# mmheyer/a3-reliable-transport

Hardware: AMD Instinct MI355X
Metric: GiB/s CRC-32 over device-resident 1456-B payloads; % of HBM read roofline (higher is better)
Workload: dtype u8

## Files before the change

a3-reliable-transport_amd/csrc/crc32_kernels.hip:

```cpp
#include <hip/hip_runtime.h>

#include <algorithm>
#include <atomic>
#include <cstdarg>
#include <cstdint>
#include <cstdio>
#include <cstdlib>
#include <cstring>
#include <mutex>
#include <type_traits>
#include <unordered_map>
#include <string>
#include <vector>

#include "crc32_math.hpp"
#include "wtp_crc32.h"

namespace wtp {

constexpr int kG = 16;
constexpr int kBraids = 4 * kG;
constexpr uint32_t kBraidBlock = 4 * kBraids;
#ifndef WTP_PC_S
#define WTP_PC_S 64
// ... 131 lines not shown
            for (int k = 0; k < PER; ++k)
                v[k] = sets[(k * THREADS) >> 11].g[stag_fill_word((uint32_t(k * THREADS) + threadIdx.x) & 2047u)];
        }
    }
    __device__ __forceinline__ void store(char *lds, const StagSet (&sets)[NS]) const {
        if constexpr (kX4) {
#pragma unroll
            for (int k = 0; k < PER; ++k) {
                const uint32_t sidx = (uint32_t(k * THREADS) + threadIdx.x) & 511u;
                uint32_t soff;
                if constexpr (THREADS <= 512) {
                    soff = sets[(k * THREADS) >> 9].off;
                } else {
                    const uint32_t si = (uint32_t(k * THREADS) + threadIdx.x) >> 9;
                    soff = sets[0].off;
#pragma unroll
                    for (int i = 1; i < NS; ++i) soff = si == uint32_t(i) ? sets[i].off : soff;
                }
                const uint32_t base = soff + (sidx >> 3) * 1024u + ((sidx >> 1) & 3u) * 32u + (sidx & 1u) * 16u;
#pragma unroll
                for (uint32_t i = 0; i < 4; ++i)
                    *reinterpret_cast<u32x4 *>(lds + base + i * 256u) = u32x4{v[k][i], v[k][i], v[k][i], v[k][i]};
            }
        } else {
#pragma unroll
            for (int k = 0; k < PER; ++k) {
                const uint32_t j = (uint32_t(k * THREADS) + threadIdx.x) & 2047u;
                *reinterpret_cast<u32x4 *>(lds + sets[(k * THREADS) >> 11].off + stag_fill_off(j)) =
                    u32x4{v[k], v[k], v[k], v[k]};
            }
        }
    }
};
template <int NS, int THREADS>
__device__ __forceinline__ void fill_stag_batch(char *lds, const StagSet (&sets)[NS]) {
    StagFill<NS, THREADS> f;
    f.load(sets);
    f.store(lds, sets);
}

__device__ __forceinline__ uint32_t braid_lead(uintptr_t st, uint32_t len, uint32_t frame) {
    const uint32_t l128 = uint32_t(st & 127u), l64 = uint32_t(st & 63u);
    return l128 + len <= frame ? l128 : (l64 + len <= frame ? l64 : frame - len);
}

__device__ __forceinline__ uint32_t xor3(uint32_t a, uint32_t b, uint32_t c) {
    return __builtin_amdgcn_bitop3_b32(a, b, c, 0x96);
}

template <uint32_t OFF>
__device__ __forceinline__ uint32_t stag_apply3x(const char *lds, const uint32_t (&key)[4], const uint32_t (&sel)[4],
                                                 uint32_t x, uint32_t w) {
    const uint32_t a0 = __builtin_amdgcn_perm(x, key[0], sel[0]);
    const uint32_t a1 = __builtin_amdgcn_perm(x, key[1], sel[1]);
    const uint32_t a2 = __builtin_amdgcn_perm(x, key[2], sel[2]);
    const uint32_t a3 = __builtin_amdgcn_perm(x, key[3], sel[3]);
    return xor3(xor3(lds_rd(lds, a0 + OFF), lds_rd(lds, a1 + OFF), lds_rd(lds, a2 + OFF)), lds_rd(lds, a3 + OFF), w);
}

template <uint32_t OFF>
__device__ __forceinline__ uint32_t stag_apply3(const char *lds, const uint32_t (&key)[4], const uint32_t (&sel)[4],
                                                uint32_t x) {
    const uint32_t a0 = __builtin_amdgcn_perm(x, key[0], sel[0]);
    const uint32_t a1 = __builtin_amdgcn_perm(x, key[1], sel[1]);
    const uint32_t a2 = __builtin_amdgcn_perm(x, key[2], sel[2]);
    const uint32_t a3 = __builtin_amdgcn_perm(x, key[3], sel[3]);
    return xor3(lds_rd(lds, a0 + OFF), lds_rd(lds, a1 + OFF), lds_rd(lds, a2 + OFF)) ^ lds_rd(lds, a3 + OFF);
}

__device__ __forceinline__ uint32_t nib_apply(const char *lds, uint32_t base, uint32_t v) {
    uint32_t l[8];
#pragma unroll
    for (uint32_t i = 0; i < 8; ++i) l[i] = lds_rd(lds, base + 64u * i + 4u * __builtin_amdgcn_ubfe(v, 4 * i, 4));
    return xor3(xor3(l[0], l[1], l[2]), xor3(l[3], l[4], l[5]), l[6] ^ l[7]);
}

__device__ __forceinline__ void rotate_prio(uint32_t x) {
    switch (x & 3u) {
    case 0: __builtin_amdgcn_s_setprio(0); break;
    case 1: __builtin_amdgcn_s_setprio(1); break;
    case 2: __builtin_amdgcn_s_setprio(2); break;
    default: __builtin_amdgcn_s_setprio(3); break;
    }
}

struct CrcBEpi {
    static constexpr bool kCopy = false;
    static constexpr bool kFixup = false;
    static constexpr int kThreads = 512;
    static constexpr int kDepth = 2;
    static constexpr int kDiag = 0;
    static constexpr int kBound = 1024;
    static constexpr int kLoadAux = 2;
    static constexpr bool kHold = false;
    static constexpr const char *kName = "CrcBEpi";
    __device__ __forceinline__ uint32_t lead(uint64_t, uint32_t st, uint32_t len, uint32_t frame) const {
        return braid_lead(st, len, frame);
    }
    uint32_t *out;
    uint32_t cinit;
    struct Pre {};
    __device__ __forceinline__ void pre(uint64_t, Pre &) const {}
    __device__ __forceinline__ bool listed(bool, const Pre &) const { return false; }
    __device__ __forceinline__ void put(uint64_t p, uint32_t v, bool on, const Pre &) const {
        if (on) out[p] = v ^ cinit;
    }
};
struct CrcHoldBEpi : CrcBEpi {
    static constexpr bool kHold = true;
    static constexpr const char *kName = "CrcHoldBEpi";
};
struct VerifyBEpi {
    static constexpr bool kHold = false;
    static constexpr const char *kName = "VerifyBEpi";
    static constexpr bool kCopy = false;
    static constexpr bool kFixup = true;
    static constexpr int kThreads = 512;
    static constexpr int kDepth = 2;
    static constexpr int kDiag = 0;
    static constexpr int kBound = 1024;
    static constexpr int kLoadAux = 2;
    __device__ __forceinline__ uint32_t lead(uint64_t, uint32_t st, uint32_t len, uint32_t frame) const {
        return braid_lead(st, len, frame);
    }
    const uint32_t *rl;
    const uint8_t *ring;
    uint64_t stride;
    uint8_t *ok;
    uint32_t *crc;
    uint32_t *status;
    uint32_t cinit;
    uint64_t n;
    uint32_t full;
    struct Pre {
        uint32_t r, h;
    };
    __device__ __forceinline__ void pre(uint64_t p, Pre &q) const {
        typedef const __attribute__((address_space(1))) uint32_t gu32;
        const uint64_t pc = p < n ? p : n - 1;
        q.r = ((gu32 *)rl)[pc];
        q.h = *(gu32 *)((gu8 *)ring + pc * stride + 12);
    }
    __device__ __forceinline__ bool listed(bool on, const Pre &q) const { return on && q.r != full; }
    __device__ __forceinline__ void put(uint64_t p, uint32_t v, bool on, const Pre &q) const {
        if (!on) return;
        const uint32_t c = v ^ cinit;
        const bool mine = q.r == full;
        ok[p] = mine && bswap32(q.h) == c ? 1 : 0;
        if (crc) crc[p] = mine ? c : 0u;
    }
};

__device__ __forceinline__ __amdgpu_buffer_rsrc_t make_rsrc(const void *base, uint32_t nbytes);
#ifndef WTP_BUILD_THREADS
#define WTP_BUILD_THREADS 128
#endif
#ifndef WTP_BUILD_DIAG
#define WTP_BUILD_DIAG 0
#endif
#ifndef WTP_BUILD_DEPTH
#define WTP_BUILD_DEPTH 2
#endif
#ifndef WTP_BUILD_SAUX
#define WTP_BUILD_SAUX 2
#endif
#ifndef WTP_BUILD_WLEAD
#define WTP_BUILD_WLEAD 1
#endif
#ifndef WTP_BUILD_LAUX
#define WTP_BUILD_LAUX 2
#endif
#ifndef WTP_BUILD_SAUX0
#define WTP_BUILD_SAUX0 0
#endif
struct BuildBEpi {
    static constexpr bool kHold = false;
    static constexpr const char *kName = "BuildBEpi";
    static constexpr bool kCopy = true;
    static constexpr bool kFixup = false;
    static constexpr int kThreads = WTP_BUILD_THREADS;
    static constexpr int kDepth = WTP_BUILD_DEPTH;
    static constexpr int kDiag = WTP_BUILD_DIAG;
    static constexpr int kBound = WTP_BUILD_THREADS;
    static constexpr int kLoadAux = WTP_BUILD_LAUX;
    uint8_t *wire;
    uint64_t wstride;
    uint32_t seq0, len;
    uint32_t *wire_len;
    uint32_t cinit;
    struct Pre {};
    __device__ __forceinline__ void pre(uint64_t, Pre &) const {}
    __device__ __forceinline__ uint32_t lead(uint64_t p, uint32_t st, uint32_t l, uint32_t frame) const {
        if (WTP_BUILD_WLEAD) {
            const uint32_t w = (uint32_t(reinterpret_cast<uintptr_t>(wire)) + uint32_t(p) * uint32_t(wstride) + 16u) & 63u;
            if (w + l <= frame) return w;
        }
        return braid_lead(st, l, frame);
    }
    __device__ __forceinline__ __amdgpu_buffer_rsrc_t round_rsrc(uint64_t p0) const {
        return make_rsrc(wire + p0 * wstride, uint32_t(4 * wstride));
    }
    __device__ __forceinline__ void copy(__amdgpu_buffer_rsrc_t rs, uint32_t q, int32_t rel, bool valid, u32x4 w,
                                         bool row0) const {
        const uint32_t o = valid ? q * uint32_t(wstride) + 16u + uint32_t(rel) : 0x80000000u;
        if (row0)
            __builtin_amdgcn_raw_buffer_store_b128(w, rs, int(o), 0, WTP_BUILD_SAUX0);
        else
            __builtin_amdgcn_raw_buffer_store_b128(w, rs, int(o), 0, WTP_BUILD_SAUX);
    }
    __device__ __forceinline__ bool listed(bool, const Pre &) const { return false; }
    __device__ __forceinline__ void put(uint64_t p, uint32_t v, bool on, const Pre &) const {
        if (!on) return;
        const u32x4 h = {bswap32(WTP_TYPE_DATA), bswap32(seq0 + uint32_t(p)), bswap32(len), bswap32(v ^ cinit)};
        *reinterpret_cast<u32x4 *>(wire + p * wstride) = h;
        if (wire_len) wire_len[p] = 16u + len;
    }
};

__device__ __forceinline__ void verify_fixup(char *lds, const VerifyBEpi &epi, const uint32_t *gtab, uint32_t nfix,
                                             uint64_t rstep, uint32_t wave, uint32_t lane);

template <int ROWS, int DIAG = 0, class BEpi = CrcBEpi>
__global__ __launch_bounds__(BEpi::kBound) void k_fixed_braid(const uint8_t *__restrict__ base, uint32_t stride,
                                                      uint32_t len, uint64_t n, BEpi epi,
                                                      const uint32_t *__restrict__ gtab) {
    __shared__ __attribute__((aligned(16))) uint32_t lds_w[kBraidLdsWords];
    char *lds = reinterpret_cast<char *>(lds_w);
    constexpr uint32_t kGroup = 8;

    const uint32_t lane = threadIdx.x & 63u;
    const uint32_t wave = __builtin_amdgcn_readfirstlane(threadIdx.x >> 6);
    PC_PROBE(0, __builtin_amdgcn_s_memrealtime());
    const uint32_t nwave = blockDim.x >> 6;
    const uint32_t j = lane & (kG - 1);
    const uint32_t q = lane >> 4;
    const StagKeys K(lane);

    constexpr uint32_t kFrame = 256u * ROWS;
    const uint64_t rounds = (n + 3) >> 2;
    const uint64_t rstep = uint64_t(gridDim.x) * nwave;
    const uint32_t qoff = q * stride;
    gu8 *const gbase = (gu8 *)base;

    struct Round {
        u32x4 w[ROWS];
        uint32_t lead;
    };
    auto load_round = [&](uint64_t rr, Round &R) {
        const bool live = rr < rounds;
        const uint64_t p0 = rr * 4;
        gu8 *sb = gbase + (live ? p0 * stride : 0);
        const uint64_t last = live ? n - 1 - p0 : 0;
        const uint32_t nrec = !live ? 0u : (last >= 3 ? 3u * stride + len : uint32_t(last) * stride + len);
        const __amdgpu_buffer_rsrc_t rs = make_rsrc((const void *)sb, nrec);
        const uint32_t lead = (DIAG & 64) ? kFrame - len
                                          : epi.lead(p0 + q, uint32_t(reinterpret_cast<uintptr_t>((const void *)sb)) + qoff, len, kFrame);
        R.lead = lead;
        const uint32_t fo = qoff - lead + j * 16u;
#pragma unroll
        for (int i = 0; i < ROWS; ++i) {
            uint32_t o = fo + uint32_t(i) * 256u;
            if (i == 0 || i == ROWS - 1) {
                const int32_t rel = int32_t(uint32_t(i) * 256u + j * 16u) - int32_t(lead);
                o = (rel >= 0 && rel < int32_t(len)) ? o : 0x80000000u;
            }
            if (i == 0)
                R.w[i] = __builtin_bit_cast(u32x4, __builtin_amdgcn_raw_buffer_load_b128(rs, int(o), 0, (DIAG & 32) ? BEpi::kLoadAux : 0));
            else
                R.w[i] = __builtin_bit_cast(u32x4, __builtin_amdgcn_raw_buffer_load_b128(rs, int(o), 0, BEpi::kLoadAux));
        }
    };

    lchar *const xs = (lchar *)(lds + kBraidXpose + wave * 2048u);
    uint32_t k = 0;
    uint64_t rfirst = 0;
    typename BEpi::Pre pre{};
    uint32_t nfix = 0;
    constexpr bool kDump = ((BEpi::kHold && !(DIAG & 2048)) || (DIAG & 1024)) && !BEpi::kCopy && !BEpi::kFixup;
    const bool hold = kDump && nwave <= 8;
#ifndef WTP_BR_HOLD
#define WTP_BR_HOLD 16
#endif
    constexpr uint32_t kHoldG = WTP_BR_HOLD;
    static_assert(kHoldG == 4 || kHoldG == 8 || kHoldG == 16, "hold capacity");
    lchar *const rbuf = (lchar *)(lds + kBraidXpose + (8u + wave) * 2048u);
    uint32_t dgroups = 0;
    uint64_t dfirst = 0;
    auto dump = [&]() {
        if constexpr (kDump) {
            __builtin_amdgcn_wave_barrier();
            const uint64_t pb0 = 4 * dfirst, left = n > pb0 ? n - pb0 : 0;
            const __amdgpu_buffer_rsrc_t ors =
                make_rsrc(epi.out + pb0, left >= (1ull << 29) ? 0x80000000u : uint32_t(4 * left));
#pragma unroll
            for (uint32_t t = 0; t < (kHoldG * 8 + 63) / 64; ++t) {
                const uint32_t si = lane + 64u * t;
                const u32x4 v = *(const lu32x4 *)(rbuf + si * 16u);
                const uint64_t rr = dfirst + (8u * uint64_t(si >> 3) + (si & 7u)) * rstep;
                const uint64_t pb = 4 * rr;
                const uint32_t o = uint32_t(4 * (pb - pb0));
                const bool live = (si >> 3) < dgroups && rr < rounds;
                if (__builtin_amdgcn_ballot_w64(live && pb + 4 > n) == 0) {
                    __builtin_amdgcn_raw_buffer_store_b128(v, ors, live ? int(o) : int(0x80000000u), 0, 0);
                } else {
                    __builtin_amdgcn_raw_buffer_store_b32(v.x, ors, live && pb + 0 < n ? int(o) : int(0x80000000u), 0, 0);
                    __builtin_amdgcn_raw_buffer_store_b32(v.y, ors, live && pb + 1 < n ? int(o + 4) : int(0x80000000u), 0, 0);
                    __builtin_amdgcn_raw_buffer_store_b32(v.z, ors, live && pb + 2 < n ? int(o + 8) : int(0x80000000u), 0, 0);
                    __builtin_amdgcn_raw_buffer_store_b32(v.w, ors, live && pb + 3 < n ? int(o + 12) : int(0x80000000u), 0, 0);
                }
            }
            __builtin_amdgcn_wave_barrier();
            dgroups = 0;
        }
    };
    auto group_packet = [&](uint64_t g0) { return (g0 + uint64_t(lane >> 3) * rstep) * 4 + ((lane >> 1) & 3u); };

    auto flush = [&](uint64_t next_g0, bool more) {
        __builtin_amdgcn_wave_barrier();
        const u32x4 lo = *(const lu32x4 *)(xs + lane * 32u), hi = *(const lu32x4 *)(xs + lane * 32u + 16u);
        uint32_t acc = hi.w;
        acc = stag_apply3x<0>(lds, K.kB, K.sel, acc, hi.z);
        acc = stag_apply3x<0>(lds, K.kB, K.sel, acc, hi.y);
        acc = stag_apply3x<0>(lds, K.kB, K.sel, acc, hi.x);
        acc = stag_apply3x<0>(lds, K.kB, K.sel, acc, lo.w);
        acc = stag_apply3x<0>(lds, K.kB, K.sel, acc, lo.z);
        acc = stag_apply3x<0>(lds, K.kB, K.sel, acc, lo.y);
        acc = stag_apply3x<0>(lds, K.kB, K.sel, acc, lo.x);
        const uint32_t h = lane & 1u;
        {
            const uint32_t y = stag_apply3<128>(lds, K.kB, K.sel, acc);
            acc = h ? y : acc;
        }
        const uint64_t rr = rfirst + uint64_t(lane >> 3) * rstep;
        const uint64_t p = rr * 4 + ((lane >> 1) & 3u);
        const uint32_t st = uint32_t(reinterpret_cast<uintptr_t>(base)) + uint32_t(p) * stride;
        const uint32_t t = (kFrame - len - ((DIAG & 64) ? kFrame - len : epi.lead(p, st, len, kFrame))) >> 4;
        const uint32_t tmax = (kFrame - len) >> 4;
        for (uint32_t s2 = 0; s2 < tmax; ++s2) {
            const uint32_t y = stag_apply3<0>(lds, K.kB, K.sel, acc);
            acc = s2 < t ? y : acc;
        }
        acc ^= uint32_t(__builtin_amdgcn_update_dpp(0, int(acc), 0xB1, 0xF, 0xF, false));
        if (!(DIAG & 1)) acc = stag_apply3<0>(lds, K.kA, K.sel, acc);
        const bool on = h == 0 && (lane >> 3) < k && rr < rounds && p < n;
        if constexpr (kDump) {
            if (hold) {
                if (dgroups == 0) dfirst = rfirst;
                if (h == 0)
                    *(__attribute__((address_space(3))) uint32_t *)(rbuf + (dgroups * 8u + (lane >> 3)) * 16u +
                                                                     ((lane >> 1) & 3u) * 4u) = acc ^ epi.cinit;
                if (++dgroups == kHoldG) dump();
            } else if (!(DIAG & 16)) {
                epi.put(p, acc, on, pre);
            }
        } else if (!(DIAG & 16)) {
            epi.put(p, acc, on, pre);
        }
        if constexpr (BEpi::kFixup) nfix += uint32_t(__popcll(__ballot(epi.listed(on, pre))));
        if (more) epi.pre(group_packet(next_g0), pre);
        k = 0;
    };

    auto crc_round = [&](uint64_t rr, const Round &R) {
        if constexpr (BEpi::kCopy) {
            const auto crs = epi.round_rsrc(rr * 4);
            const bool qlive = rr * 4 + q < n;
#pragma unroll
            for (int i = 0; i < ROWS; ++i) {
                const int32_t rel = int32_t(uint32_t(i) * 256u + j * 16u) - int32_t(R.lead);
                const bool in = (i == 0 || i == ROWS - 1) ? (rel >= 0 && rel < int32_t(len)) : true;
                epi.copy(crs, q, rel, in && qlive, R.w[i], i == 0);
            }
        }
        uint32_t b0 = R.w[0].x, b1 = R.w[0].y, b2 = R.w[0].z, b3 = R.w[0].w;
#pragma unroll
        for (int i = 1; i < ROWS; ++i) {
            const u32x4 w = R.w[i];
            if (DIAG & 1) {
                b0 = (b0 ^ w.x) + (b0 >> 3);
                b1 = (b1 ^ w.y) + (b1 >> 3);
                b2 = (b2 ^ w.z) + (b2 >> 3);
                b3 = (b3 ^ w.w) + (b3 >> 3);
                continue;
            }
            b0 = stag_apply3x<0>(lds, K.kA, K.sel, b0, w.x);
            b1 = stag_apply3x<0>(lds, K.kA, K.sel, b1, w.y);
            b2 = stag_apply3x<0>(lds, K.kA, K.sel, b2, w.z);
            b3 = stag_apply3x<0>(lds, K.kA, K.sel, b3, w.w);
        }
        uint32_t v;
        if (DIAG & 2) {
            v = xor3(b0, b1, b2) ^ b3;
        } else {
            v = stag_apply3x<128>(lds, K.kA, K.sel, b3, b2);
            v = stag_apply3x<128>(lds, K.kA, K.sel, v, b1);
            v = stag_apply3x<128>(lds, K.kA, K.sel, v, b0);
        }
        if (k == 0) rfirst = rr;
        *(__attribute__((address_space(3))) uint32_t *)(xs + k * 256u + lane * 4u) = v;
        if (++k == kGroup) flush(rr + rstep, true);
    };

    uint64_t r = uint64_t(blockIdx.x) * nwave + wave;
    Round A, B;
    const StagSet sets[4] = {{gtab + OFF_BRAID, 0u},
                             {gtab + OFF_INV + 0 * 1024, 128u},
                             {gtab + OFF_INV + 2 * 1024, 65536u},
                             {gtab + OFF_INV + 5 * 1024, 65536u + 128u}};
    constexpr int kT = BEpi::kThreads;
    StagFill<4, kT> fill;
    const bool batched = blockDim.x == kT;
#ifndef WTP_BR_PROLOGUE_DIAG
#define WTP_BR_PROLOGUE_DIAG 0
#endif
    if (batched && WTP_BR_PROLOGUE_DIAG == 0) fill.load(sets);
    if constexpr (WTP_BR_PROLOGUE_DIAG == 1)
        for (int kk = 0; kk < fill.PER; ++kk) fill.v[kk] = threadIdx.x + kk;
    epi.pre(group_packet(r), pre);
    load_round(r, A);
    PC_PROBE(1, __builtin_amdgcn_s_memrealtime());
    if (WTP_BR_PROLOGUE_DIAG == 2) {
    } else if (batched) {
        fill.store(lds, sets);
    } else {
        for (int q2 = 0; q2 < 4; ++q2) fill_stag(lds, sets[q2].off >> 16, (sets[q2].off >> 7) & 1u, sets[q2].g);
    }
    PC_PROBE(2, __builtin_amdgcn_s_memrealtime());
    __syncthreads();
    PC_PROBE(3, __builtin_amdgcn_s_memrealtime());

    uint32_t prio_round = wave >> 2;
    if constexpr (BEpi::kDepth == 3) {
        Round C;
        load_round(r + rstep, B);
        while (r < rounds) {
            if (!(DIAG & 4)) rotate_prio(++prio_round);
            load_round(r + 2 * rstep, C);
            crc_round(r, A);
            r += rstep;
            if (r >= rounds) break;
            load_round(r + 2 * rstep, A);
            crc_round(r, B);
            r += rstep;
            if (r >= rounds) break;
            load_round(r + 2 * rstep, B);
            crc_round(r, C);
            r += rstep;
        }
    } else {
        while (r < rounds) {
            if (!(DIAG & 4)) rotate_prio(++prio_round);
            load_round(r + rstep, B);
            crc_round(r, A);
            if (WTP_PROBE && prio_round == (wave >> 2) + 1) PC_PROBE(4, __builtin_amdgcn_s_memrealtime());
            r += rstep;
            if (r >= rounds) break;
            load_round(r + rstep, A);
            crc_round(r, B);
            r += rstep;
        }
    }
    if (k) flush(0, false);
    if constexpr (kDump) {
        if (dgroups) dump();
    }
    PC_PROBE(5, __builtin_amdgcn_s_memrealtime());
    if constexpr (BEpi::kFixup) verify_fixup(lds, epi, gtab, nfix, rstep, wave, lane);
}

__device__ __forceinline__ __amdgpu_buffer_rsrc_t make_rsrc(const void *base, uint32_t nbytes);
struct MetaRaw {
    uint64_t a;
    uint32_t b, c, d;
};
constexpr uint32_t kRunBad = 1u, kCutBad = 2u;
struct RangeDesc {
    uint64_t begin, end, rebase;
    uint32_t nbytes, bad;
};
static_assert(sizeof(RangeDesc) == 32, "RangeDesc");
template <class P>
constexpr bool kDevRange = requires { requires P::kDevRange; };
struct CrcEpi {
    static constexpr const char *kName = "CrcEpi";
    uint32_t *out;
    uint32_t n;
    __device__ __forceinline__ void rebase(uint64_t first, uint32_t cnt) {
        out += first;
        n = cnt;
    }
    __device__ __forceinline__ void put(uint64_t p, uint32_t crc, bool, uint32_t, bool on) const {
        __builtin_amdgcn_raw_buffer_store_b32(crc, make_rsrc(out, 4 * n), on ? int(4 * p) : int(0x80000000u), 0, 0);
    }
};
struct VerifyEpi {
    static constexpr const char *kName = "VerifyEpi";
    uint8_t *ok;
    uint32_t *crc;
    uint32_t n;
    __device__ __forceinline__ void put(uint64_t p, uint32_t c, bool valid, uint32_t want, bool on) const {
        const bool good = valid && want == c;
        __builtin_amdgcn_raw_buffer_store_b8(uint8_t(good ? 1 : 0), make_rsrc(ok, n), on ? int(p) : int(0x80000000u),
                                             0, 0);
        __builtin_amdgcn_raw_buffer_store_b32(valid ? c : 0u, make_rsrc(crc, crc ? 4 * n : 0u),
                                              on ? int(4 * p) : int(0x80000000u), 0, 0);
    }
};

__device__ __forceinline__ __amdgpu_buffer_rsrc_t make_rsrc(const void *base, uint32_t nbytes) {
    return __builtin_amdgcn_make_buffer_rsrc(const_cast<void *>(base), (short)0, (int)nbytes, 0x00020000);
}
__device__ __forceinline__ u32x4 buf_ld16(__amdgpu_buffer_rsrc_t r, uint32_t off) {
    return __builtin_bit_cast(u32x4, __builtin_amdgcn_raw_buffer_load_b128(r, (int)off, 0, 0));
}

#ifndef WTP_PC_THREADS
#define WTP_PC_THREADS 1024
#endif
constexpr uint32_t kPcThreads = WTP_PC_THREADS, kPcLogT = __builtin_ctz(kPcThreads), kPcWaves = kPcThreads / 64;
constexpr uint32_t kPcWords = uint32_t(kPieceS) / 4;
constexpr uint32_t kPcNOps = kPieceS == 64 ? 5 : 6;
constexpr uint32_t kPcOps = 65536;
constexpr uint32_t kPcHinit = kPcOps + kPcNOps * kOpBytes;
#ifndef WTP_PC_SPLIT
// ... 394 lines not shown
                const uint64_t k64 = uint64_t(0xFFFFFFFFu) << (uint32_t(t) & 63u);
                const uint32_t keep = (i & 1) ? uint32_t(k64 >> 32) : uint32_t(k64);
                if ((i & 1) == 0)
                    ca = stag_apply3<0>(lds, K.kA, K.sel, __builtin_amdgcn_bitop3_b32(ca, wd, keep, 0x78));
                else if (i < 15)
                    cb = stag_apply3<0>(lds, K.kA, K.sel, __builtin_amdgcn_bitop3_b32(cb, wd, keep, 0x78));
                else
                    cb = nib_apply(lds, kPcNib4, __builtin_amdgcn_bitop3_b32(cb, wd, keep, 0x78));
            }
            c = ca ^ cb;
        }
        const uint32_t hw = lds_rd(lds, kPcHinit + 4u * uint32_t(kPieceS - (vf < 0 ? 0 : vf)));
        c ^= gp == 0u ? hw : 0u;

        uint32_t W = c;
        {
            const uint32_t u = __shfl_up(W, 1);
            if constexpr (kPieceS == 64) {
                if (lp >= 1u && lane >= 1u) W = stag_apply3x<128>(lds, K.kA, K.sel, u, W);
            } else {
                if (lp >= 1u && lane >= 1u) W = op_apply_fold(lds, kPcOps, u, W);
            }
        }
#pragma unroll
        for (uint32_t dd = 2, o = 0; dd < 64; dd <<= 1, ++o) {
            const bool need = lp >= dd && lane >= dd;
            if (__builtin_amdgcn_ballot_w64(need) == 0) break;
            const uint32_t u = __shfl_up(W, dd);
            if (need) W = op_apply_fold(lds, kPcOps + (o + kPcNOps - 5) * kOpBytes, u, W);
        }
        epi.put(pout, W ^ 0xFFFFFFFFu, pvalid, paux, active && gp == pkk - 1);
        carry = partial ? __builtin_amdgcn_readlane(W, tl) : 0u;
        skip = partial ? last_gp + 1 : 0u;
        p0 = uniform64(p0n);
        if (WTP_PROBE && nrounds == 0) PC_PROBE(4, __builtin_amdgcn_s_memrealtime());
        ++nrounds;
        if constexpr (Prov::kVarLen && WTP_PC_LAG) {
            done += total;
            const uint32_t left = wpieces > done ? wpieces - done : 0u;
            const uint32_t simd = wave & 3u;
            typedef __attribute__((address_space(3))) uint32_t lu32w;
            if (lane == 0) *(lu32w *)((lchar *)lds + kPcRem + 4u * (4u * simd + (wave >> 2))) = left;
            const uint32_t other = *(const lu32w *)((lchar *)lds + kPcRem + 16u * simd + 4u * (lane & 3u));
            rotate_prio(uint32_t(__popcll(__builtin_amdgcn_ballot_w64(lane < kPcWaves / 4u && other < left))));
        } else {
            rotate_prio(nrounds + (wave >> 2));
        }
    }
    PC_PROBE(5, __builtin_amdgcn_s_memrealtime());
    PC_PROBE(6, nrounds);
    PC_PROBE(7, hi - lo);
}

template <int THREADS>
struct PcTables {
    static constexpr uint32_t kOpQ = kPcNOps * 256, kOpPer = (kOpQ + THREADS - 1) / THREADS;
    StagFill<2, THREADS> fill;
    u32x4 q[kOpPer];
    uint32_t hv;
    u32x4 n4;
    __device__ __forceinline__ static void sets(const uint32_t *gtab, StagSet (&s)[2]) {
        s[0] = {gtab + (WTP_PC_SPLIT ? OFF_S8 : OFF_S4), 0u};
        s[1] = {gtab + (kPieceS == 64 ? OFF_FWD : OFF_X64), 128u};
    }
    __device__ __forceinline__ void load(const uint32_t *gtab) {
        StagSet ss[2];
        sets(gtab, ss);
        fill.load(ss);
        const u32x4 *src = reinterpret_cast<const u32x4 *>(gtab + OFF_FWD + 1024 * (6 - kPcNOps));
#pragma unroll
        for (uint32_t k = 0; k < kOpPer; ++k) {
            const uint32_t i = threadIdx.x + k * THREADS;
            q[k] = src[i < kOpQ ? i : 0];
        }
        hv = gtab[OFF_HINIT + (threadIdx.x <= kPieceS ? threadIdx.x : 0)];
        if constexpr (WTP_PC_SPLIT)
            n4 = reinterpret_cast<const u32x4 *>(gtab + OFF_NIB + 128 * 10)[threadIdx.x & 31u];
    }
    __device__ __forceinline__ void store(char *lds, const uint32_t *gtab) const {
        StagSet ss[2];
        sets(gtab, ss);
        fill.store(lds, ss);
        u32x4 *dst = reinterpret_cast<u32x4 *>(lds + kPcOps);
#pragma unroll
        for (uint32_t k = 0; k < kOpPer; ++k) {
            const uint32_t i = threadIdx.x + k * THREADS;
            if (i < kOpQ) dst[i] = q[k];
        }
        if (threadIdx.x <= kPieceS) reinterpret_cast<uint32_t *>(lds + kPcHinit)[threadIdx.x] = hv;
        if constexpr (WTP_PC_SPLIT)
            if (threadIdx.x < 32u) reinterpret_cast<u32x4 *>(lds + kPcNib4)[threadIdx.x] = n4;
    }
};

template <class Prov, class Epi>
__global__ __launch_bounds__(kPcThreads) void k_pieces(const uint8_t *__restrict__ base_in, uint32_t nbytes_in,
                                                 Prov prov_in, uint64_t n_in, Epi epi_in,
                                                 const uint32_t *__restrict__ gtab, uint32_t *__restrict__ status) {
    __shared__ __attribute__((aligned(16))) uint32_t lds_w[kPcLdsWords];
    char *lds = reinterpret_cast<char *>(lds_w);
    Prov prov = prov_in;
    Epi epi = epi_in;
    const uint8_t *base = base_in;
    uint32_t nbytes = nbytes_in;
    uint64_t n = n_in;
    if constexpr (kDevRange<Prov>) {
        if (!prov.bind(base, nbytes, n, epi)) return;
    }
    const uint32_t nw = blockDim.x >> 6;
    const uint64_t tw = uint64_t(gridDim.x) * nw, w0 = uint64_t(blockIdx.x) * nw;
    const uint64_t g0 = n * w0 / tw, g1 = n * (w0 + nw) / tw;
    if (g0 == g1) return;
    const uint32_t lane = threadIdx.x & 63u;
    const uint32_t wave = __builtin_amdgcn_readfirstlane(threadIdx.x >> 6);
    const __amdgpu_buffer_rsrc_t rs = make_rsrc(base, nbytes);
    PC_PROBE(0, __builtin_amdgcn_s_memrealtime());
    WaveSplit split;
    PcTables<kPcThreads> tb;
    tb.load(gtab);
    if constexpr (Prov::kVarLen) split.load(prov, g0, g1);
    PC_PROBE(1, __builtin_amdgcn_s_memrealtime());
    tb.store(lds, gtab);
    uint64_t lo, hi;
    uint32_t wpieces = 0;
    if constexpr (Prov::kVarLen) {
        split.finish(prov, g0, g1, lds, wave, lane, lo, hi, wpieces);
    } else {
        lo = n * (w0 + wave) / tw;
        hi = n * (w0 + wave + 1) / tw;
    }
    MetaRaw raw{};
    if (lo < hi) pieces_meta(prov, lo, hi, lane, raw, rs);
    __syncthreads();
    PC_PROBE(2, __builtin_amdgcn_s_memrealtime());

    pieces_loop(lds, rs, prov, epi, lo, hi, wpieces, status, wave, lane, raw);
}

constexpr uint32_t kVfWaves = 8;
constexpr uint32_t kVfList = kPcStage + kVfWaves * kPcSlot;
constexpr uint32_t kVfCap = (kPcFlags - kVfList) / 4;
constexpr uint32_t kVfCtl = (kPcLdsWords * 4 + 15) & ~15u;
constexpr uint32_t kVfPer = 8;
constexpr uint32_t kVfPass = kVfWaves * 64 * kVfPer;
static_assert(kVfPass <= kVfCap && kVfCtl + 64 <= kBraidLdsWords * 4, "verify fix-up LDS");

#ifndef WTP_AB_BUILD
static_assert(WTP_PC_S == 64 && WTP_PC_THREADS == 1024 && WTP_PC_LEN128 == 1 && WTP_PC_LAG == 1 && WTP_PC_DMA == 1 &&
                  WTP_PC_TAILCLAMP == 0 && WTP_PC_SPLIT == 0,
              "product build: piece-kernel knobs must keep their shipped values");
static_assert(WTP_BR_PROLOGUE_DIAG == 0 && WTP_PROBE == 0, "product build: no probe / prologue ablation");
static_assert(WTP_BR_HOLD == 16 && WTP_FILL_X4 == 1 && WTP_FILL_X4_PC == 1,
              "product build: held results every 16 flushes, 16-B table fill (braided and piece kernels)");
static_assert(WTP_BUILD_THREADS == 128 && WTP_BUILD_DIAG == 0 && WTP_BUILD_DEPTH == 2 && WTP_BUILD_SAUX == 2 &&
                  WTP_BUILD_WLEAD == 1 && WTP_BUILD_LAUX == 2 && WTP_BUILD_SAUX0 == 0,
              "product build: fused-builder knobs must keep their shipped values");
#endif

typedef __attribute__((address_space(3))) uint32_t lu32;

struct LdsIdxDgramProv {
    static constexpr const char *kName = "LdsIdxDgramProv";
    static constexpr bool kVarLen = false;
    static constexpr bool kIndexed = true;
    static constexpr bool kGroupLoad = false;
    uint64_t stride;
    const uint32_t *__restrict__ rl;
    const lu32 *list;
    __device__ __forceinline__ void load(uint64_t p, MetaRaw &r, __amdgpu_buffer_rsrc_t rs) const {
        const uint32_t idx = list[p];
        const uint32_t h = uint32_t(uint64_t(idx) * stride + 12);
        r.a = idx;
        r.b = rl[idx];
        const u32x2 w = __builtin_bit_cast(u32x2, __builtin_amdgcn_raw_buffer_load_b64(rs, int(h), 0, 0));
        r.c = w.x;
        r.d = w.y;
    }
    __device__ __forceinline__ void decode(const MetaRaw &r, uint64_t &off, uint32_t &l, bool &ok, uint32_t &want,
                                           uint32_t &slot) const {
        const uint64_t d = r.a * stride;
        want = bswap32(r.c);
        off = d + 16;
        ok = r.b >= 16 && r.b <= stride;
        l = ok ? r.b - 16 : 0;
        slot = uint32_t(r.a);
    }
};

__device__ __forceinline__ void verify_fixup(char *lds, const VerifyBEpi &epi, const uint32_t *gtab, uint32_t nfix,
                                             uint64_t rstep, uint32_t wave, uint32_t lane) {
    lu32 *const ctl = (lu32 *)((lchar *)lds + kVfCtl);
    const uint32_t nwave = blockDim.x >> 6;
    if (lane == 0) ctl[wave] = nfix;
    __syncthreads();
    uint32_t total = 0;
    for (uint32_t w = 0; w < nwave; ++w) total += ctl[w];
    total = __builtin_amdgcn_readfirstlane(total);
    if (total == 0) return;
    typedef __attribute__((address_space(1))) uint32_t gmu32;
    gmu32 *const st = (gmu32 *)epi.status;
    if (nwave != kVfWaves) {
        if (threadIdx.x == 0) __hip_atomic_fetch_or(st, 4u, __ATOMIC_RELAXED, __HIP_MEMORY_SCOPE_AGENT);
        return;
    }
    {
        PcTables<kVfWaves * 64> tb;
        tb.load(gtab);
        tb.store(lds, gtab);
    }
    const uint64_t n = epi.n;
    const __amdgpu_buffer_rsrc_t rs = make_rsrc(epi.ring, uint32_t((n * epi.stride + 15) & ~uint64_t(15)));
    const __amdgpu_buffer_rsrc_t rr = make_rsrc(epi.rl, uint32_t(4 * n));
    lu32 *const list = (lu32 *)((lchar *)lds + kVfList);
    const LdsIdxDgramProv prov{epi.stride, epi.rl, list};
    const VerifyEpi vepi{epi.ok, epi.crc, uint32_t(n)};
    const uint64_t g0 = uint64_t(blockIdx.x) * nwave;
    uint32_t found = 0;
    for (uint64_t e0 = 0; 4 * (g0 + (e0 >> 5) * rstep) < n; e0 += kVfPass) {
        if (threadIdx.x == 0) ctl[8] = 0;
        __syncthreads();
        uint64_t pv[kVfPer];
        uint32_t rv[kVfPer];
#pragma unroll
        for (uint32_t k = 0; k < kVfPer; ++k) {
            const uint64_t e = e0 + k * (kVfWaves * 64) + threadIdx.x;
            pv[k] = 4 * (g0 + (e >> 5) * rstep) + (e & 31u);
            rv[k] = __builtin_amdgcn_raw_buffer_load_b32(rr, pv[k] < n ? int(4 * pv[k]) : int(0x80000000u), 0, 0);
        }
#pragma unroll
        for (uint32_t k = 0; k < kVfPer; ++k) {
            const bool need = pv[k] < n && rv[k] != epi.full;
            const uint64_t m = __ballot(need);
            if (m == 0) continue;
            uint32_t b = 0;
            if (lane == 0) b = __hip_atomic_fetch_add(&ctl[8], uint32_t(__popcll(m)), __ATOMIC_RELAXED,
                                                      __HIP_MEMORY_SCOPE_WORKGROUP);
            b = __builtin_amdgcn_readfirstlane(b);
            const uint32_t pos = __builtin_amdgcn_mbcnt_hi(uint32_t(m >> 32), __builtin_amdgcn_mbcnt_lo(uint32_t(m), 0u));
            if (need) list[b + pos] = uint32_t(pv[k]);
        }
        __syncthreads();
        const uint32_t c = __builtin_amdgcn_readfirstlane(ctl[8]);
        found += c;
        const uint64_t lo = uint64_t(c) * wave / kVfWaves, hi = uint64_t(c) * (wave + 1) / kVfWaves;
        MetaRaw raw{};
        if (lo < hi) pieces_meta(prov, lo, hi, lane, raw, rs);
        pieces_loop(lds, rs, prov, vepi, lo, hi, 0u, epi.status, wave, lane, raw);
        __syncthreads();
    }
    if (threadIdx.x == 0 && found != total) __hip_atomic_fetch_or(st, 2u, __ATOMIC_RELAXED, __HIP_MEMORY_SCOPE_AGENT);
}

constexpr uint32_t kStThreads = 512, kStWaves = kStThreads / 64;
constexpr uint32_t kStRound = 8192;
constexpr uint32_t kStLane = 144;
constexpr uint32_t kStSlot = 64 * kStLane;
constexpr uint32_t kStNib = 65536;
constexpr uint32_t kStSlots = kStNib + kStNibOps * 512;
constexpr uint32_t kStBal = kStSlots + kStWaves * kStSlot;
constexpr uint32_t kStLdsWords = (kStBal + (kStWaves + 1) * 8) / 4;
constexpr uint32_t kStMaxLen = 4095;
static_assert(kStLdsWords * 4 <= 163840, "k_stream LDS");


__device__ __forceinline__ uint32_t st_feed(const char *lds, lchar *slot, const StagKeys &K, uint32_t x) {
    typedef const __attribute__((address_space(3))) uint32_t lu32c;
    const uint32_t l = x >> 7, blk = (x >> 5) & 3u, t = x & 31u;
    lchar *const b = slot + l * kStLane + blk * 32u;
    uint32_t c = *(lu32c *)(slot + l * kStLane + 128u + 4u * blk);
    const u32x4 w0 = *(const lu32x4 *)b, w1 = *(const lu32x4 *)(b + 16);
    const uint32_t w[8] = {w0.x, w0.y, w0.z, w0.w, w1.x, w1.y, w1.z, w1.w};
    const uint32_t nw = t >> 2, r = t & 3u;
    const uint32_t wn = *(lu32c *)(b + 4u * nw);
#pragma unroll
    for (uint32_t k = 0; k < 7; ++k) {
        if (__ballot(k < nw) == 0) break;
        const uint32_t y = stag_apply3<0>(lds, K.kA, K.sel, c ^ w[k]);
        c = k < nw ? y : c;
    }
    const uint32_t y = r ? (c ^ wn) << (32u - 8u * r) : 0u;
    return (c >> (8u * r)) ^ stag_apply3<0>(lds, K.kA, K.sel, y);
}

template <int DUMMY = 0>
__global__ __launch_bounds__(kStThreads) void k_stream(const uint8_t *__restrict__ view, uint64_t view_bytes,
                                                     const uint64_t *__restrict__ offs,
                                                     const uint32_t *__restrict__ lens, uint64_t lead, uint64_t n,
                                                     uint32_t *__restrict__ out, const uint32_t *__restrict__ gtab,
                                                     uint32_t *__restrict__ status, const RangeDesc *__restrict__ gate,
                                                     uint32_t ngate) {
    typedef const __attribute__((address_space(1))) uint64_t gu64;
    typedef const __attribute__((address_space(1))) uint32_t gu32;
    if (gate) {
        uint32_t any = 0;
        for (uint32_t j = 0; j < ngate; ++j) any |= gate[j].bad;
        if (!any) return;
    }
    __shared__ __attribute__((aligned(16))) uint32_t lds_w[kStLdsWords];
    char *lds = reinterpret_cast<char *>(lds_w);
    const uint64_t g0 = n * blockIdx.x / gridDim.x, g1 = n * (blockIdx.x + 1) / gridDim.x;
    if (g0 == g1) return;
    const uint32_t lane = threadIdx.x & 63u;
    const uint32_t wave = __builtin_amdgcn_readfirstlane(threadIdx.x >> 6);
    auto off_of = [&](uint64_t p) { return ((gu64 *)offs)[p] + lead; };
    auto len_of = [&](uint64_t p) { return ((gu32 *)lens)[p]; };

    uint64_t *const starts = reinterpret_cast<uint64_t *>(lds + kStBal);
    const uint64_t span = g1 - g0;
// ... 979 lines not shown
```

Before: 6686.

## Rotate payload chunks across lanes so fused-builder wire stores are aligned

Adds a rotation path to the fused frame builder's copy. Payload 16-B chunks are shuffled across lanes with ds_bpermute, so each lane's buffer store lands on an aligned slot of the destination wire frame instead of an offset set by the braid lead. The wire-aligned lead selection is turned off under rotation, and the builder block size goes from 128 to 256 threads. The cost is ROWS+1 bpermute rounds per row group plus an extra store row, in exchange for better-aligned write coalescing.

```diff
diff --git a/a3-reliable-transport_amd/csrc/crc32_kernels.hip b/a3-reliable-transport_amd/csrc/crc32_kernels.hip
--- a/a3-reliable-transport_amd/csrc/crc32_kernels.hip
+++ b/a3-reliable-transport_amd/csrc/crc32_kernels.hip
@@ -307,8 +307,11 @@
 };
 
 __device__ __forceinline__ __amdgpu_buffer_rsrc_t make_rsrc(const void *base, uint32_t nbytes);
+#ifndef WTP_BUILD_ROT
+#define WTP_BUILD_ROT 1
+#endif
 #ifndef WTP_BUILD_THREADS
-#define WTP_BUILD_THREADS 128
+#define WTP_BUILD_THREADS (WTP_BUILD_ROT ? 256 : 128)
 #endif
 #ifndef WTP_BUILD_DIAG
 #define WTP_BUILD_DIAG 0
@@ -345,8 +348,9 @@
     uint32_t cinit;
     struct Pre {};
     __device__ __forceinline__ void pre(uint64_t, Pre &) const {}
+    static constexpr bool kRot = WTP_BUILD_ROT != 0;
     __device__ __forceinline__ uint32_t lead(uint64_t p, uint32_t st, uint32_t l, uint32_t frame) const {
-        if (WTP_BUILD_WLEAD) {
+        if (WTP_BUILD_WLEAD && !kRot) {
             const uint32_t w = (uint32_t(reinterpret_cast<uintptr_t>(wire)) + uint32_t(p) * uint32_t(wstride) + 16u) & 63u;
             if (w + l <= frame) return w;
         }
@@ -362,6 +366,47 @@
             __builtin_amdgcn_raw_buffer_store_b128(w, rs, int(o), 0, WTP_BUILD_SAUX0);
         else
             __builtin_amdgcn_raw_buffer_store_b128(w, rs, int(o), 0, WTP_BUILD_SAUX);
+    }
+    __device__ __forceinline__ uint32_t rot_d(uint64_t p, uint32_t l) const {
+        const uint32_t a = ((uint32_t(reinterpret_cast<uintptr_t>(wire)) + uint32_t(p) * uint32_t(wstride)) & 127u) >> 4;
+        return (a + 1u - l) & 7u;
+    }
+    template <int ROWS>
+    __device__ __forceinline__ void rot_move(uint64_t p, uint32_t lane, uint32_t lead_b, const u32x4 (&w)[ROWS],
+                                             u32x4 (&m)[ROWS + 1]) const {
+        const uint32_t j = lane & 15u, d = rot_d(p, lead_b >> 4);
+        const bool prev = j + d >= 16u;
+        const int from = int(((lane & 48u) | ((j - d) & 15u)) << 2);
+#pragma unroll
+        for (int i = 0; i <= ROWS; ++i) {
+            u32x4 v = w[i < ROWS ? i : ROWS - 1];
+            if (i > 0 && i < ROWS) {
+                v.x = prev ? w[i - 1].x : v.x;
+                v.y = prev ? w[i - 1].y : v.y;
+                v.z = prev ? w[i - 1].z : v.z;
+                v.w = prev ? w[i - 1].w : v.w;
+            }
+            m[i].x = uint32_t(__builtin_amdgcn_ds_bpermute(from, int(v.x)));
+            m[i].y = uint32_t(__builtin_amdgcn_ds_bpermute(from, int(v.y)));
+            m[i].z = uint32_t(__builtin_amdgcn_ds_bpermute(from, int(v.z)));
+            m[i].w = uint32_t(__builtin_amdgcn_ds_bpermute(from, int(v.w)));
+        }
+    }
+    template <int ROWS>
+    __device__ __forceinline__ void rot_store(__amdgpu_buffer_rsrc_t rs, uint64_t p, uint32_t lane, uint32_t lead_b,
+                                              bool live, const u32x4 (&m)[ROWS + 1]) const {
+        const uint32_t q = lane >> 4, j = lane & 15u, l = lead_b >> 4;
+        const int32_t k0 = int32_t(j) - int32_t(rot_d(p, l) + l), nch = int32_t(len >> 4);
+        const uint32_t o0 = q * uint32_t(wstride) + 16u;
+#pragma unroll
+        for (int i = 0; i <= ROWS; ++i) {
+            const int32_t k = k0 + 16 * i;
+            const uint32_t o = live && k >= 0 && k < nch ? o0 + 16u * uint32_t(k) : 0x80000000u;
+            if (i == 0)
+                __builtin_amdgcn_raw_buffer_store_b128(m[i], rs, int(o), 0, WTP_BUILD_SAUX0);
+            else
+                __builtin_amdgcn_raw_buffer_store_b128(m[i], rs, int(o), 0, WTP_BUILD_SAUX);
+        }
     }
     __device__ __forceinline__ bool listed(bool, const Pre &) const { return false; }
     __device__ __forceinline__ void put(uint64_t p, uint32_t v, bool on, const Pre &) const {
@@ -520,11 +565,17 @@
         if constexpr (BEpi::kCopy) {
             const auto crs = epi.round_rsrc(rr * 4);
             const bool qlive = rr * 4 + q < n;
-#pragma unroll
-            for (int i = 0; i < ROWS; ++i) {
-                const int32_t rel = int32_t(uint32_t(i) * 256u + j * 16u) - int32_t(R.lead);
-                const bool in = (i == 0 || i == ROWS - 1) ? (rel >= 0 && rel < int32_t(len)) : true;
-                epi.copy(crs, q, rel, in && qlive, R.w[i], i == 0);
+            if constexpr (BEpi::kRot) {
+                u32x4 moved[ROWS + 1];
+                epi.template rot_move<ROWS>(rr * 4 + q, lane, R.lead, R.w, moved);
+                epi.template rot_store<ROWS>(crs, rr * 4 + q, lane, R.lead, qlive, moved);
+            } else {
+#pragma unroll
+                for (int i = 0; i < ROWS; ++i) {
+                    const int32_t rel = int32_t(uint32_t(i) * 256u + j * 16u) - int32_t(R.lead);
+                    const bool in = (i == 0 || i == ROWS - 1) ? (rel >= 0 && rel < int32_t(len)) : true;
+                    epi.copy(crs, q, rel, in && qlive, R.w[i], i == 0);
+                }
             }
         }
         uint32_t b0 = R.w[0].x, b1 = R.w[0].y, b2 = R.w[0].z, b3 = R.w[0].w;
@@ -1225,8 +1276,8 @@
 static_assert(WTP_BR_PROLOGUE_DIAG == 0 && WTP_PROBE == 0, "product build: no probe / prologue ablation");
 static_assert(WTP_BR_HOLD == 16 && WTP_FILL_X4 == 1 && WTP_FILL_X4_PC == 1,
               "product build: held results every 16 flushes, 16-B table fill (braided and piece kernels)");
-static_assert(WTP_BUILD_THREADS == 128 && WTP_BUILD_DIAG == 0 && WTP_BUILD_DEPTH == 2 && WTP_BUILD_SAUX == 2 &&
-                  WTP_BUILD_WLEAD == 1 && WTP_BUILD_LAUX == 2 && WTP_BUILD_SAUX0 == 0,
+static_assert(WTP_BUILD_THREADS == 256 && WTP_BUILD_DIAG == 0 && WTP_BUILD_DEPTH == 2 && WTP_BUILD_SAUX == 2 &&
+                  WTP_BUILD_WLEAD == 1 && WTP_BUILD_LAUX == 2 && WTP_BUILD_SAUX0 == 0 && WTP_BUILD_ROT == 1,
               "product build: fused-builder knobs must keep their shipped values");
 #endif
 
```

Result: no change. 6690 (median of 6 runs) (+0.1%).
